# kpreid/all-is-cubes

Hardware: AMD Instinct MI355X
Metric: Mrays/s (higher is better)
Workload: dtype f64

## Files before the change

### all_is_cubes_amd/abi.py

```python
from __future__ import annotations

import ctypes as C
import math
from pathlib import Path
from typing import Optional

import numpy as np

_PKG = Path(__file__).resolve().parent
LIB_PATH = _PKG / "libaic_hip.so"

AIC_OK = 0
ERR_NAMES = {1: "AIC_ERR_INVALID", 2: "AIC_ERR_NO_DEVICE", 3: "AIC_ERR_OOM", 4: "AIC_ERR_DEVICE", 5: "AIC_ERR_UNSUPPORTED"}
LAYER_WORLD, LAYER_UI = 0, 1
MAX_IN_FLIGHT = 32
FLAW_UNSUPPORTED, FLAW_NO_BLOOM = 1, 2
FRAME_COUNTERS, FRAME_AUX, FRAME_PIXEL_CENTERS, FRAME_OUT_LINEAR, FRAME_OUT_COLORBUF, FRAME_NO_FEEDBACK = 1, 2, 4, 8, 16, 32
FRAME_BLOOM = 64
FRAME_OUT_SPLIT = 512
RAYS_NO_SKY, RAYS_DEVICE = 128, 256
MAX_RAYS = 2048 * 65535
PIXELS_DEVICE, PIXELS_IN_PLACE = 1, 2
MAX_PIXELS = 2048 * 65535
REPROJECT_KEEP_SPLATS = 1
# ... 35 lines not shown
        t |= ((int(super_shift) + 1) & 31) << TUNE_SUPER_SHIFT
    if variant is not None:
        t |= (int(variant) & 3) << TUNE_VARIANT_SHIFT
    return t

ABI_SYMBOLS = [
    "aic_abi_version", "aic_create", "aic_destroy", "aic_last_error", "aic_device_name", "aic_upload_space",
    "aic_clear_space", "aic_update_cubes", "aic_update_light_volume", "aic_replace_block", "aic_replace_blocks", "aic_compact", "aic_set_options", "aic_set_depth_transform",
    "aic_render", "aic_render_submit", "aic_render_wait", "aic_render_submit_batch", "aic_render_wait_batch", "aic_trace_patches", "aic_trace_rays", "aic_trace_pixels", "aic_pixel_order", "aic_reproject_split", "aic_reproject_geometry", "aic_pick_pixels", "aic_stale_rects", "aic_pick_stale", "aic_pick_stale_cubes", "aic_probe_stale_cube_rects", "aic_find_block_cubes", "aic_pick_stale_blocks", "aic_present_split", "aic_present_geometry", "aic_present_split_lines", "aic_present_lines_scratch", "aic_cursor_wireframe", "aic_cursor_raycast", "aic_set_text_font", "aic_text_geometry", "aic_text_layout", "aic_present_split_text", "aic_export_split", "aic_export_size", "aic_exposure_init", "aic_exposure_rays", "aic_sample_luminance", "aic_exposure_advance", "aic_partition_rows", "aic_assemble_strips", "aic_assemble_strips_async", "aic_assemble_strips_on", "aic_read_aux", "aic_synchronize", "aic_stream", "aic_wait_event", "aic_stream_wait_frame",
    "aic_probe_raycast", "aic_probe_light_lut", "aic_probe_powf", "aic_probe_expf", "aic_probe_bloom",
    "aic_ortho_image_size", "aic_render_orthographic",
    "aic_evaluate_light", "aic_evaluate_light_submit", "aic_evaluate_light_wait", "aic_evaluate_light_poll", "aic_light_cubes_changed", "aic_light_changed_count", "aic_light_changed_take", "aic_read_light_volume", "aic_read_light_cubes", "aic_light_chart", "aic_probe_derived", "aic_probe_log2f", "aic_probe_cube_grid",
    "aic_create_multi", "aic_destroy_multi", "aic_multi_device_count", "aic_multi_context", "aic_multi_last_error", "aic_multi_upload_space",
    "aic_multi_clear_space", "aic_multi_update_cubes", "aic_multi_update_light_volume", "aic_multi_evaluate_light", "aic_multi_light_cubes_changed", "aic_multi_replace_blocks", "aic_multi_set_options", "aic_multi_set_depth_transform",
    "aic_multi_render", "aic_multi_render_submit", "aic_multi_render_wait",
]


class AicError(RuntimeError):

    def __init__(self, code: int, message: str):
        super().__init__(f"{ERR_NAMES.get(code, code)}: {message}")
        self.code = code


class BlockDesc(C.Structure):
    _fields_ = [("resolution", C.c_int32), ("vlo", C.c_int32 * 3), ("vsize", C.c_int32 * 3), ("vox_off", C.c_uint32),
                ("pal_off", C.c_uint32), ("pal_len", C.c_uint32), ("flags", C.c_uint32), ("reserved", C.c_int32)]


class LightParams(C.Structure):
# ... 362 lines not shown
        lib.aic_last_error.argtypes = [C.c_void_p]
        lib.aic_stream.restype = C.c_void_p
        lib.aic_stream.argtypes = [C.c_void_p]
        lib.aic_partition_rows.restype = C.c_uint32
        lib.aic_partition_rows.argtypes = [C.c_uint32, C.POINTER(Partition)]
        lib.aic_upload_space.argtypes = [C.c_void_p, C.c_int, C.POINTER(SpaceDesc)]
        lib.aic_clear_space.argtypes = [C.c_void_p, C.c_int]
        lib.aic_compact.argtypes = [C.c_void_p, C.c_int]
        lib.aic_update_cubes.argtypes = [C.c_void_p, C.c_int, C.c_uint32, C.c_void_p, C.c_void_p, C.c_void_p]
        lib.aic_update_light_volume.argtypes = [C.c_void_p, C.c_int, C.c_void_p]
        lib.aic_replace_block.argtypes = [C.c_void_p, C.c_int, C.c_uint32, C.POINTER(BlockDesc), C.c_void_p, C.c_void_p]
        lib.aic_replace_blocks.argtypes = [C.c_void_p, C.c_int, C.c_uint32, C.c_void_p, C.c_void_p, C.c_void_p, C.c_void_p]
        lib.aic_set_options.argtypes = [C.c_void_p, C.c_int, C.POINTER(Options)]
        lib.aic_set_depth_transform.argtypes = [C.c_void_p, C.POINTER(C.c_double)]
        lib.aic_render.argtypes = [C.c_void_p, C.POINTER(FrameDesc), C.c_void_p, C.c_int, C.POINTER(FrameInfo)]
        lib.aic_render_submit.argtypes = [C.c_void_p, C.POINTER(FrameDesc), C.c_void_p, C.c_uint32]
        lib.aic_render_wait.argtypes = [C.c_void_p, C.c_uint32, C.POINTER(FrameInfo)]
        lib.aic_render_submit_batch.argtypes = [C.c_void_p, C.c_uint32, C.POINTER(FrameDesc), C.POINTER(C.c_void_p), C.c_uint32]
        lib.aic_render_wait_batch.argtypes = [C.c_void_p, C.c_uint32, C.c_uint32, C.POINTER(FrameInfo)]
        lib.aic_trace_patches.argtypes = [C.c_void_p, C.POINTER(FrameDesc), C.c_uint32, C.c_void_p, C.c_void_p, C.c_void_p, C.POINTER(FrameInfo)]
        lib.aic_trace_rays.argtypes = [C.c_void_p, C.c_int, C.c_uint32, C.c_void_p, C.c_uint32, C.c_float, C.c_void_p, C.c_void_p, C.POINTER(FrameInfo)]
        lib.aic_trace_pixels.argtypes = [C.c_void_p, C.POINTER(FrameDesc), C.c_uint32, C.c_void_p, C.c_uint32, C.c_void_p, C.c_void_p, C.POINTER(FrameInfo)]
        lib.aic_reproject_split.argtypes = [C.c_void_p, C.POINTER(ReprojectDesc), C.c_void_p, C.c_void_p, C.POINTER(ReprojectInfo)]
        lib.aic_pick_pixels.argtypes = [C.c_void_p, C.POINTER(PickDesc), C.c_void_p, C.c_void_p, C.POINTER(PickInfo)]
        lib.aic_pick_stale.argtypes = [C.c_void_p, C.POINTER(StaleDesc), C.c_void_p, C.c_void_p, C.c_void_p, C.POINTER(StaleInfo)]
        lib.aic_light_changed_count.argtypes = [C.c_void_p, C.c_int, C.POINTER(C.c_uint64), C.c_void_p]
        lib.aic_light_changed_take.argtypes = [C.c_void_p, C.c_int, C.c_uint32, C.c_void_p, C.POINTER(C.c_uint32)]
        lib.aic_pick_stale_cubes.argtypes = [C.c_void_p, C.POINTER(StaleCubesDesc), C.c_void_p, C.c_void_p, C.c_void_p, C.POINTER(StaleCubesInfo)]
        lib.aic_probe_stale_cube_rects.argtypes = [C.c_void_p, C.POINTER(StaleCubesDesc), C.c_void_p]
        lib.aic_find_block_cubes.argtypes = [C.c_void_p, C.c_int, C.c_uint32, C.c_void_p, C.c_uint32, C.c_void_p, C.POINTER(BlockCubesInfo)]
# ... 270 lines not shown
        out = np.zeros(rows * frame.width * 3, np.uint32) if split else np.zeros((rows, frame.width, 4), np.float32 if floats else np.uint8)
        info = FrameInfo()
        try:
            self._check(self._lib.aic_render(self._h, C.byref(frame), _ptr(out), 0, C.byref(info)))
        finally:
            frame.flags = keep_flags
        aux = None
        if want_aux:
            aux = np.zeros((rows, frame.width), PIXEL_AUX_DTYPE)
            if aux.size:
                self._check(self._lib.aic_read_aux(self._h, _ptr(aux), aux.size))
        if split:
            return {**split_planes(out, rows, frame.width), "info": info, "aux": aux}
        return {"rgba8": out, "info": info, "aux": aux}

    def render_to_device(self, frame: FrameDesc, device_ptr: int) -> FrameInfo:
        info = FrameInfo()
        self._check(self._lib.aic_render(self._h, C.byref(frame), C.c_void_p(device_ptr), 1, C.byref(info)))
        return info

    def trace_patches(self, frame: FrameDesc, rects, want_aux: bool = False):
        r = np.ascontiguousarray(rects, np.float64).reshape(-1, 4)
        out = np.zeros((len(r), 4), np.float32 if frame.flags & (FRAME_OUT_LINEAR | FRAME_OUT_COLORBUF) else np.uint8)
        aux = np.zeros(len(r), PIXEL_AUX_DTYPE) if want_aux else None
        info = FrameInfo()
        self._check(self._lib.aic_trace_patches(self._h, C.byref(frame), len(r), _ptr(r), _ptr(out), _ptr(aux), C.byref(info)))
        return {"rgba8": out, "aux": aux, "info": info}

    def trace_rays(self, layer: int, rays, include_sky: bool = True, flags: int = 0, exposure: float = 1.0, want_aux: bool = False):
        r = np.ascontiguousarray(rays, np.float64).reshape(-1, 6)
# ... 500 lines not shown
```

### all_is_cubes_amd/csrc/aic_abi.cpp

```cpp

#include <hip/hip_runtime.h>

#include <chrono>
#include <cmath>
#include <condition_variable>
#include <mutex>
#include <thread>
#include <cstdio>
#include <cstdlib>
#include <cstring>
#include <initializer_list>
#include <string>
#include <utility>
#include <vector>

#include "../../include/aic_hip.h"
#include "aic_bloom.h"
#include "aic_ctx.h"
#include "aic_device.h"
#include "aic_encode.h"
#include "aic_launch.h"

using namespace aic;

// ... 303 lines not shown
        aic_ctx::FrameSlot &fs = c->slots[i];
        if (fs.stream) (void)hipStreamSynchronize(fs.stream);
        for (auto &sb : fs.sub) sb.release();
        fs.ray_cold.release(); fs.edges.release();
        if (fs.ev0) (void)hipEventDestroy(fs.ev0);
        if (fs.ev1) (void)hipEventDestroy(fs.ev1);
        if (fs.ev2) (void)hipEventDestroy(fs.ev2);
        fs.tile_static.release(); fs.queue_static.release();
        if (i > 0 && fs.stream) (void)hipStreamDestroy(fs.stream);
    }
    for (auto &l : c->layers) l.release();
    c->lut.release(); c->srgb_thr.release(); c->srgb_buckets.release(); c->out.release(); c->aux.release(); c->staging.release(); c->ortho_views.release(); c->reproject_scratch.release(); c->pick_scratch.release(); c->stale_scratch.release(); c->stale_cubes_scratch.release(); c->stale_blocks_scratch.release(); c->stale_blocks_boxes.release(); c->present_scratch.release(); c->lines_scratch.release();
    c->text_atlas.release(); c->text_codes.release(); c->export_counts.release(); c->exposure_scratch.release(); c->cursor_scratch.release();
    for (hipEvent_t ev : c->stale_blocks_ev)
        if (ev) (void)hipEventDestroy(ev);
    if (c->dump) std::fclose(c->dump);
    if (c->upload_stream) (void)hipStreamDestroy(c->upload_stream);
    if (c->stream) (void)hipStreamDestroy(c->stream);
    delete c;
}

const char *aic_last_error(const aic_ctx *c) { return c ? c->err.c_str() : "no context"; }

int aic_device_name(const aic_ctx *c, char *buf, uint32_t buf_len) {
    if (!c || !buf || !buf_len) return AIC_ERR_INVALID;
    std::snprintf(buf, buf_len, "%s", c->devname);
    return AIC_OK;
}

int aic_upload_space(aic_ctx *c, int layer, const aic_space_desc *s) {
// ... 550 lines not shown
```

### all_is_cubes_amd/csrc/aic_ctx.h

```cpp
#pragma once

#include <hip/hip_runtime.h>

#include <chrono>
#include <condition_variable>
#include <cstdio>
#include <initializer_list>
#include <mutex>
#include <string>
#include <thread>
#include <vector>

#include "../../include/aic_hip.h"
#include "aic_device.h"

namespace aic {

template <typename T>
struct DevBuf {
    T *p = nullptr;
    size_t n = 0;
    size_t cap = 0;
    hipError_t ensure(size_t count, bool keep = false, hipStream_t stream = nullptr) {
        if (count <= cap) { n = count; return hipSuccess; }
        size_t new_cap = count + count / 4 + 16;
        T *np_ = nullptr;
        hipError_t e = hipMalloc((void **)&np_, new_cap * sizeof(T));
        if (e != hipSuccess) return e;
        if (keep && p && cap) {
// ... 155 lines not shown
    } ljob;
    struct Switches {
        int tile = 0, macro = 0;
        bool feedback = true;
        bool wait_whole_stream = false;
        uint32_t tiles_per_wave = 0;
        std::string wave_prof;
        bool lines_clear_keys = false;
    } sw;
    DevBuf<unsigned char> stale_scratch;
    DevBuf<unsigned char> cursor_scratch;
    DevBuf<unsigned char> stale_cubes_scratch;
    DevBuf<unsigned char> stale_blocks_scratch;
    DevBuf<int32_t> stale_blocks_boxes;
    hipEvent_t stale_blocks_ev[2] = {nullptr, nullptr};
};

namespace aic {

extern thread_local std::string *tl_err_sink;
int fail(aic_ctx *c, int code, const char *what, hipError_t e = hipSuccess);
int hip_fail(aic_ctx *c, const char *what, hipError_t e);
inline int reject(aic_ctx *c, const char *who, const char *why) { return fail(c, AIC_ERR_INVALID, (std::string(who) + ": " + why).c_str()); }
#define HIP_TRY(ctx, expr)                                    \
    do {                                                      \
        hipError_t e_ = (expr);                               \
        if (e_ != hipSuccess) return hip_fail(ctx, #expr, e_); \
    } while (0)

inline bool valid_layer(int l) { return l == AIC_LAYER_WORLD || l == AIC_LAYER_UI; }

aic_options default_options();
enum DumpTag : uint32_t { DUMP_UPLOAD = 1, DUMP_CLEAR = 2, DUMP_CUBES = 3, DUMP_LIGHT = 4, DUMP_BLOCK = 5, DUMP_OPTIONS = 6, DUMP_FRAME = 7 };
struct DumpPart { const void *p; size_t n; };
void dump_record(aic_ctx *c, uint32_t tag, uint32_t layer, std::initializer_list<DumpPart> parts);
int take_light_spare(aic_ctx *c, Layer &l, int layer, size_t n, int *index);
int quiesce(aic_ctx *c);
int light_job_finish(aic_ctx *c);
constexpr uint32_t kVisibleBitsWords = 2048;
int light_visible_bits(aic_ctx *c, Layer &l, hipStream_t stream, std::vector<uint32_t> *bits);

}
```

### all_is_cubes_amd/csrc/aic_frame.cpp

```cpp

#include <hip/hip_runtime.h>

#include <algorithm>
#include <chrono>
#include <cmath>
#include <cstdio>
#include <cstring>
#include <utility>
#include <vector>

#include "../../include/aic_hip.h"
#include "aic_bloom.h"
#include "aic_ctx.h"
#include "aic_device.h"
#include "aic_launch.h"

using namespace aic;

namespace {

void fill_dev_layer(const Layer &l, const aic_camera &cam, DevLayer *d) {
    std::memset(d, 0, sizeof(*d));
    d->present = l.present ? 1 : 0;
    d->pool = l.pool.p;
// ... 636 lines not shown
}
int finish_listed(aic_ctx *c, uint32_t n, bool to_host, aic_pixel_aux *aux, aic_frame_info *info) {
    const int rc = wait_frame(c, 0, info, to_host);
    if (rc != AIC_OK) return rc;
    if (aux && to_host) HIP_TRY(c, hipMemcpy(aux, c->aux.p, (size_t)n * sizeof(aic_pixel_aux), hipMemcpyDeviceToHost));
    if (info) info->rows_rendered = n;
    return AIC_OK;
}

int submit_in_world_seat(aic_ctx *c, int layer, const aic_frame_desc *f, uint32_t *target, bool allow_aux, const Traced &what) {
    Traced seated = what;
    seated.world_seat = layer;
    return submit_frame(c, f, target, 0, allow_aux, seated);
}

}

extern "C" {

int aic_render(aic_ctx *c, const aic_frame_desc *f, void *out_rgba8, int out_is_device, aic_frame_info *info) {
    if (!c || !f) return fail(c, AIC_ERR_INVALID, "aic_render: bad argument");
    if (info) std::memset(info, 0, sizeof(*info));
    if (const int rc = begin_on_slot0(c, "aic_render")) return rc;
    uint32_t *target = (uint32_t *)out_rgba8;
    const size_t px_words = (f->flags & (AIC_FRAME_OUT_LINEAR | AIC_FRAME_OUT_COLORBUF)) ? 4 : ((f->flags & AIC_FRAME_OUT_SPLIT) ? 3 : 1);
    if (!out_is_device && out_rgba8) {
        const aic_partition part = normalised_partition(*f);
        const size_t npix = (size_t)f->width * (part.part < part.n_parts ? aic_partition_rows(f->height, &part) : 0);
        hipError_t e;
        if (npix && (e = c->out.ensure(npix * px_words)) != hipSuccess) return hip_fail(c, "alloc output", e);
        target = c->out.p;
    }
    int rc = submit_frame(c, f, target, 0, true);
    if (rc != AIC_OK) return rc;
    if (!out_is_device && c->slots[0].npix)
        HIP_TRY(c, hipMemcpyAsync(out_rgba8, c->out.p, c->slots[0].npix * px_words * 4, hipMemcpyDeviceToHost, c->slots[0].stream));
    return wait_frame(c, 0, info, !out_is_device);
}

int aic_ortho_image_size(const int32_t lo[3], const int32_t size[3], int resolution, uint32_t *width, uint32_t *height) {
    if (!lo || !size || !width || !height || !valid_ortho_resolution(resolution) || size[0] < 0 || size[1] < 0 || size[2] < 0) return AIC_ERR_INVALID;
    DevOrthoView v[5];
    multi_ortho(resolution, lo, size, v, width, height);
// ... 212 lines not shown
```

### all_is_cubes_amd/host/aic_host.cpp

```cpp
#include "aic_host.hpp"

#include <algorithm>
#include <cmath>
#include <cstdio>
#include <cstring>

namespace aic::host {

#define MM(t, r, c) ((t).m[((r)-1) * 4 + ((c)-1)])

Mat4 Mat4::then(const Mat4 &o) const {
    Mat4 out;
    for (int r = 1; r <= 4; r++)
        for (int c = 1; c <= 4; c++)
            MM(out, r, c) = MM(*this, r, 1) * MM(o, 1, c) + MM(*this, r, 2) * MM(o, 2, c) + MM(*this, r, 3) * MM(o, 3, c) +
                            MM(*this, r, 4) * MM(o, 4, c);
    return out;
}

bool Mat4::inverse(Mat4 *out) const {
    const double m11 = MM(*this, 1, 1), m12 = MM(*this, 1, 2), m13 = MM(*this, 1, 3), m14 = MM(*this, 1, 4);
    const double m21 = MM(*this, 2, 1), m22 = MM(*this, 2, 2), m23 = MM(*this, 2, 3), m24 = MM(*this, 2, 4);
    const double m31 = MM(*this, 3, 1), m32 = MM(*this, 3, 2), m33 = MM(*this, 3, 3), m34 = MM(*this, 3, 4);
    const double m41 = MM(*this, 4, 1), m42 = MM(*this, 4, 2), m43 = MM(*this, 4, 3), m44 = MM(*this, 4, 4);
// ... 424 lines not shown
    char buf[256];
    const double per = (width && height) ? (double)cubes_traced / ((double)width * height) : 0.0;
    std::snprintf(buf, sizeof(buf), "Traced %llu cubes, %.1f cubes/pixel in %u\xC3\x97%u image", (unsigned long long)cubes_traced, per, width, height);
    return buf;
}

static_assert(sizeof(PackedLight) == 4, "PackedLight is a 4-byte texel");

HipRtRenderer::HipRtRenderer(std::shared_ptr<StandardCameras> cameras, SizePolicy size_policy, int device_id)
    : cameras_(std::move(cameras)), size_policy_(std::move(size_policy)), world_camera_(GraphicsOptions(), Viewport::with_scale(1.0, 1, 1)),
      ui_camera_(GraphicsOptions(), Viewport::with_scale(1.0, 1, 1)) {
    if (!cameras_) throw std::invalid_argument("cameras must not be null");
    int status = 0;
    ctx_ = aic_create(device_id, &status);
    if (!ctx_) throw RenderError(status, status == AIC_ERR_NO_DEVICE ? "no usable HIP device (MI355X required)" : "aic_create failed");
}
HipRtRenderer::~HipRtRenderer() { aic_destroy(ctx_); }

void HipRtRenderer::check(int rc, const char *what) {
    if (rc != AIC_OK) throw RenderError(rc, std::string(what) + ": " + aic_last_error(ctx_));
}
Viewport HipRtRenderer::modified_viewport() const { return size_policy_ ? size_policy_(cameras_->viewport) : cameras_->viewport; }
std::string HipRtRenderer::device_name() const {
    char buf[256];
    aic_device_name(ctx_, buf, sizeof(buf));
    return buf;
}
void *HipRtRenderer::stream() const { return aic_stream(ctx_); }

void HipRtRenderer::upload_full(int layer, const Space &space) {
    aic_space_desc d;
    std::memset(&d, 0, sizeof(d));
// ... 157 lines not shown
}

static ImageInfo to_info(const aic_frame_info &fi, uint32_t w, uint32_t h) {
    ImageInfo i;
    i.cubes_traced = fi.cubes_traced; i.n_outer = fi.n_outer; i.n_inner = fi.n_inner; i.n_hits = fi.n_hits; i.n_light = fi.n_light;
    i.kernel_ms = fi.kernel_ms; i.total_ms = fi.total_ms; i.width = w; i.height = h; i.rows_rendered = fi.rows_rendered;
    return i;
}

Rendering HipRtRenderer::draw_rgba(const std::string &info_text) {
    aic_frame_desc f = make_frame();
    if (bloom_) f.flags |= AIC_FRAME_BLOOM;
    Rendering r;
    r.width = f.width;
    r.height = f.height;
    r.data.assign((size_t)f.width * f.height * 4, 0);
    aic_frame_info fi;
    check(aic_render(ctx_, &f, r.data.data(), 0, &fi), "aic_render");
    r.info = to_info(fi, f.width, f.height);
    if (fi.flaws & AIC_FLAW_UNSUPPORTED) r.flaws |= Flaws::UNSUPPORTED;
    if (fi.flaws & AIC_FLAW_NO_BLOOM) r.flaws |= Flaws::NO_BLOOM;
    if (had_cursor_) r.flaws |= Flaws::NO_CURSOR;
    if (!info_text.empty() && world_camera_.options().debug_info_text && f.width && f.height) {
        uint8_t black[4], white[4];
        const float k0[3] = {0.f, 0.f, 0.f}, k1[3] = {1.f, 1.f, 1.f};
        const float paint_exposure = cam_override_ ? cam_override_exposure_ : world_camera_.exposure();
        encode_paint(world_camera_, paint_exposure, k0, black);
        encode_paint(world_camera_, paint_exposure, k1, white);
        draw_info_text(r.data.data(), f.width, f.height, black, white, info_text);
    }
    return r;
}

// ... 662 lines not shown
```

### all_is_cubes_amd/host/aic_host.hpp

```cpp
#pragma once

#include <array>
#include <cstdint>
#include <cstring>
#include <functional>
#include <limits>
#include <memory>
#include <optional>
#include <set>
#include <stdexcept>
#include <string>
#include <vector>

#include "../../include/aic_hip.h"

namespace aic::host {

struct Vec3 {
    double x = 0, y = 0, z = 0;
};
struct Quat {
    double i = 0, j = 0, k = 0, r = 1;
};
struct Mat4 {
// ... 210 lines not shown

struct ImageInfo {
    uint64_t cubes_traced = 0;
    uint64_t n_outer = 0, n_inner = 0, n_hits = 0, n_light = 0;
    float kernel_ms = 0, total_ms = 0;
    uint32_t width = 0, height = 0, rows_rendered = 0;
    std::string status_text() const;
};
struct SplitRendering {
    uint32_t width = 0, height = 0;
    std::vector<uint16_t> color;
    std::vector<float> depth;
    uint16_t flaws = 0;
    ImageInfo info;
};
struct Rendering {
    uint32_t width = 0, height = 0;
    std::vector<uint8_t> data;
    uint16_t flaws = 0;
    ImageInfo info;
};

void draw_info_text(uint8_t *rgba, uint32_t width, uint32_t height, const uint8_t outline[4], const uint8_t foreground[4], const std::string &text);
constexpr uint32_t kInfoTextCell[3] = {9, 18, 1};
std::vector<uint8_t> info_text_font_atlas();
void encode_paint(const class Camera &camera, float exposure, const float rgb[3], uint8_t out[4]);

struct UiViewState {
    std::shared_ptr<Space> space;
    ViewTransform view_transform;
    float backdrop[4] = {0, 0, 0, 0};
    GraphicsOptions graphics_options;
};
// ... 166 lines not shown
  private:
    struct LayerState {
        std::shared_ptr<Space> space;
        std::shared_ptr<SpaceRendererTodo> todo;
        GraphicsOptions options;
        bool options_valid = false;
    };
    bool sync_space(int layer, const std::shared_ptr<Space> &space, const GraphicsOptions &options);
    void upload_full(int layer, const Space &space);
    void check(int rc, const char *what);
    aic_present_desc present_desc(uint32_t out_width, uint32_t out_height, uint32_t flags) const;
    aic_frame_desc make_frame() const;
    std::shared_ptr<StandardCameras> cameras_;
    SizePolicy size_policy_;
    aic_ctx *ctx_ = nullptr;
    LayerState layers_[2];
    bool cam_override_ = false;
    double cam_override_inv_[16] = {0};
    float cam_override_exposure_ = 1.0f;
    bool had_cursor_ = false;
    std::vector<aic_line_vertex> cursor_lines_;
    aic_lines_desc lines_desc(const std::vector<aic_line_vertex> *lines) const;
    bool text_font_set_ = false;
    std::vector<uint8_t> text_codes_;
    aic_text_desc text_desc(const std::string &info_text);
    bool bloom_ = false;
    uint64_t pick_cursor_ = 0, pick_skip_unknown_ = 0;
    uint64_t pick_skip_stale_ = 0;
    std::vector<std::array<int32_t, 6>> changed_boxes_;
    std::vector<std::array<int32_t, 6>> changed_cube_boxes_;
// ... 78 lines not shown
```

### all_is_cubes_amd/host/py_module.cpp

```cpp
#include <pybind11/functional.h>
#include <pybind11/numpy.h>
#include <pybind11/pybind11.h>
#include <pybind11/stl.h>

#include <cstring>

#include "aic_host.hpp"

namespace py = pybind11;
using namespace aic::host;

static Vec3 v3(const std::array<double, 3> &a) { return Vec3{a[0], a[1], a[2]}; }
static std::array<double, 3> a3(const Vec3 &v) { return {v.x, v.y, v.z}; }
static py::array_t<double> mat(const Mat4 &m) {
    py::array_t<double> out({4, 4});
    std::memcpy(out.mutable_data(), m.m, sizeof(m.m));
    return out;
}

PYBIND11_MODULE(_host, m) {
    m.doc() = "C++ host mirror of the all-is-cubes raytracer interface above the MI355X C ABI";

    py::register_exception<RenderError>(m, "RenderError");

// ... 192 lines not shown
                      [](UiViewState &u, const std::array<float, 4> &b) { for (int i = 0; i < 4; i++) u.backdrop[i] = b[i]; });
    py::class_<StandardCameras, std::shared_ptr<StandardCameras>>(m, "StandardCameras")
        .def(py::init([]() { return std::make_shared<StandardCameras>(); }))
        .def_readwrite("graphics_options", &StandardCameras::graphics_options).def_readwrite("viewport", &StandardCameras::viewport)
        .def_readwrite("world_space", &StandardCameras::world_space).def_readwrite("world_view_transform", &StandardCameras::world_view_transform)
        .def_readwrite("measured_exposure", &StandardCameras::measured_exposure).def_readwrite("ui", &StandardCameras::ui);

    py::class_<ImageInfo>(m, "ImageInfo")
        .def_readonly("cubes_traced", &ImageInfo::cubes_traced).def_readonly("n_outer", &ImageInfo::n_outer).def_readonly("n_inner", &ImageInfo::n_inner)
        .def_readonly("n_hits", &ImageInfo::n_hits).def_readonly("n_light", &ImageInfo::n_light).def_readonly("kernel_ms", &ImageInfo::kernel_ms)
        .def_readonly("total_ms", &ImageInfo::total_ms).def_readonly("width", &ImageInfo::width).def_readonly("height", &ImageInfo::height)
        .def_readonly("rows_rendered", &ImageInfo::rows_rendered).def("status_text", &ImageInfo::status_text);
    py::class_<Rendering>(m, "Rendering")
        .def_readonly("width", &Rendering::width).def_readonly("height", &Rendering::height).def_readonly("flaws", &Rendering::flaws)
        .def_readonly("info", &Rendering::info)
        .def_property_readonly("data", [](const Rendering &r) {
            py::array_t<uint8_t> a({(py::ssize_t)r.height, (py::ssize_t)r.width, (py::ssize_t)4});
            if (!r.data.empty()) std::memcpy(a.mutable_data(), r.data.data(), r.data.size());
            return a;
        });

    py::class_<SplitRendering>(m, "SplitRendering")
        .def_readonly("width", &SplitRendering::width).def_readonly("height", &SplitRendering::height).def_readonly("flaws", &SplitRendering::flaws)
        .def_readonly("info", &SplitRendering::info)
        .def_property_readonly("color_f16_bits", [](const SplitRendering &r) {
            py::array_t<uint16_t> a({(py::ssize_t)r.height, (py::ssize_t)r.width, (py::ssize_t)4});
            if (!r.color.empty()) std::memcpy(a.mutable_data(), r.color.data(), r.color.size() * 2);
            return a;
        })
        .def_property_readonly("depth", [](const SplitRendering &r) {
            py::array_t<float> a({(py::ssize_t)r.height, (py::ssize_t)r.width});
            if (!r.depth.empty()) std::memcpy(a.mutable_data(), r.depth.data(), r.depth.size() * 4);
            return a;
        });
// ... 391 lines not shown
```

### include/aic_hip.h

```cpp
#ifndef AIC_HIP_H
#define AIC_HIP_H

#include <stdint.h>

#ifdef __cplusplus
extern "C" {
#endif

#define AIC_ABI_VERSION 3

#define AIC_OK 0
#define AIC_ERR_INVALID 1
#define AIC_ERR_NO_DEVICE 2
#define AIC_ERR_OOM 3
#define AIC_ERR_DEVICE 4
#define AIC_ERR_UNSUPPORTED 5

#define AIC_LAYER_WORLD 0
#define AIC_LAYER_UI 1

#define AIC_FLAW_UNSUPPORTED 1u
#define AIC_FLAW_NO_BLOOM 2u

#define AIC_BLOCK_ONE 1u
// ... 118 lines not shown

int aic_upload_space(aic_ctx *ctx, int layer, const aic_space_desc *space);
int aic_clear_space(aic_ctx *ctx, int layer);
int aic_update_cubes(aic_ctx *ctx, int layer, uint32_t n, const int32_t *xyz, const uint16_t *block_index,
                     const uint8_t *light);
int aic_update_light_volume(aic_ctx *ctx, int layer, const uint8_t *light);
int aic_replace_block(aic_ctx *ctx, int layer, uint32_t index, const aic_block_desc *desc, const uint16_t *voxels,
                      const float *palette);
int aic_replace_blocks(aic_ctx *ctx, int layer, uint32_t n, const uint32_t *indices, const aic_block_desc *descs,
                       const uint16_t *const *voxels, const float *const *palettes);
int aic_compact(aic_ctx *ctx, int layer);
int aic_set_options(aic_ctx *ctx, int layer, const aic_options *options);
int aic_set_depth_transform(aic_ctx *ctx, const double zw[4]);

int aic_render(aic_ctx *ctx, const aic_frame_desc *frame, void *out_rgba8, int out_is_device, aic_frame_info *info);
#define AIC_MAX_IN_FLIGHT 32u
int aic_render_submit(aic_ctx *ctx, const aic_frame_desc *frame, void *out_device, uint32_t slot);
int aic_render_wait(aic_ctx *ctx, uint32_t slot, aic_frame_info *info);
int aic_render_submit_batch(aic_ctx *ctx, uint32_t n_frames, const aic_frame_desc *frames, void *const *out_devices, uint32_t slot);
int aic_render_wait_batch(aic_ctx *ctx, uint32_t slot, uint32_t n_frames, aic_frame_info *infos);
int aic_trace_patches(aic_ctx *ctx, const aic_frame_desc *frame, uint32_t n, const double *rects, void *out_rgba8,
                      aic_pixel_aux *aux, aic_frame_info *info);
#define AIC_RAYS_NO_SKY 128u
#define AIC_RAYS_DEVICE 256u
int aic_trace_rays(aic_ctx *ctx, int layer, uint32_t n, const double *rays, uint32_t flags, float exposure, void *out, aic_pixel_aux *aux,
                   aic_frame_info *info);
#define AIC_PIXELS_DEVICE 1u
#define AIC_PIXELS_IN_PLACE 2u
int aic_trace_pixels(aic_ctx *ctx, const aic_frame_desc *frame, uint32_t n, const uint32_t *pixels, uint32_t mode, void *out, aic_pixel_aux *aux,
                     aic_frame_info *info);
// ... 329 lines not shown
```

### rust/all-is-cubes-hip/src/ffi.rs

```rust
#![allow(non_camel_case_types, missing_docs, clippy::missing_safety_doc)]

use core::ffi::{c_char, c_int, c_void};

pub const AIC_ABI_VERSION: c_int = 3;
pub const AIC_OK: c_int = 0;
pub const AIC_ERR_INVALID: c_int = 1;
pub const AIC_ERR_NO_DEVICE: c_int = 2;
pub const AIC_ERR_OOM: c_int = 3;
pub const AIC_ERR_DEVICE: c_int = 4;
pub const AIC_ERR_UNSUPPORTED: c_int = 5;
pub const AIC_LAYER_WORLD: c_int = 0;
pub const AIC_LAYER_UI: c_int = 1;
pub const AIC_BLOCK_ONE: u32 = 1;
pub const AIC_BLOCK_AIR: u32 = 2;
pub const AIC_BLOCK_UNSELECTABLE: u32 = 4;
pub const AIC_BLOCK_VOXEL_SELECTABLE: u32 = 8;
pub const AIC_FLAW_UNSUPPORTED: u32 = 1;
pub const AIC_FLAW_NO_BLOOM: u32 = 2;
pub const AIC_FRAME_COUNTERS: u32 = 1;
pub const AIC_FRAME_AUX: u32 = 2;
pub const AIC_FRAME_PIXEL_CENTERS: u32 = 4;
pub const AIC_FRAME_OUT_LINEAR: u32 = 8;
pub const AIC_FRAME_OUT_COLORBUF: u32 = 16;
pub const AIC_FRAME_NO_FEEDBACK: u32 = 32;
// ... 6 lines not shown
pub const AIC_REPROJECT_KEEP_SPLATS: u32 = 1;
pub const AIC_REPROJECT_MAX_LEVELS: u32 = 12;
pub const AIC_PRESENT_OUT_F16: u32 = 1;
pub const AIC_PRESENT_MAX_PIXELS: u64 = 2147483648;
pub const AIC_LINES_DEVICE: u32 = 1;
pub const AIC_TEXT_DEVICE: u32 = 1;
pub const AIC_LINES_MAX: u32 = 1048576;
pub const AIC_STALE_DEPTH_TEST: u32 = 1;
pub const AIC_STALE_MAX_RECTS: u32 = 4096;
pub const AIC_STALE_DEPTH_BEHIND: u32 = 2;
pub const AIC_CURSOR_MAX_LINES: u32 = 28;
pub const AIC_CURSOR_NO_BLOCK: u32 = 0xFFFF_FFFF;
pub const AIC_EXPOSURE_SAMPLES: u32 = 100;
pub const AIC_EXPOSURE_RAYS: u32 = 10;
pub const AIC_MAX_IN_FLIGHT: u32 = 32;
pub const AIC_MULTI_MAX_IN_FLIGHT: u32 = 8;
pub const AIC_TUNE_QUEUES_SHIFT: u32 = 0;
pub const AIC_TUNE_SUPER_SHIFT: u32 = 4;
pub const AIC_TUNE_VARIANT_SHIFT: u32 = 9;
pub const AIC_VARIANT_AUTO: u32 = 0;
pub const AIC_VARIANT_PLAIN: u32 = 1;
pub const AIC_VARIANT_EXCHANGING: u32 = 2;
pub const AIC_VARIANT_RECORDING: u32 = 3;
pub const AIC_LIGHT_HOOK_SESSION: i32 = 1;
pub const AIC_LIGHT_HOOK_POOL_SHIFT: i32 = 8;

#[repr(C)]
#[derive(Clone, Copy, Debug, Default)]
pub struct aic_block_desc {
    pub resolution: i32,
// ... 425 lines not shown
    pub fn aic_create(device_id: c_int, status: *mut c_int) -> *mut aic_ctx;
    pub fn aic_destroy(ctx: *mut aic_ctx);
    pub fn aic_last_error(ctx: *const aic_ctx) -> *const c_char;
    pub fn aic_abi_version() -> c_int;
    pub fn aic_device_name(ctx: *const aic_ctx, buf: *mut c_char, buf_len: u32) -> c_int;
    pub fn aic_upload_space(ctx: *mut aic_ctx, layer: c_int, space: *const aic_space_desc) -> c_int;
    pub fn aic_clear_space(ctx: *mut aic_ctx, layer: c_int) -> c_int;
    pub fn aic_update_cubes(ctx: *mut aic_ctx, layer: c_int, n: u32, xyz: *const i32, block_index: *const u16, light: *const u8) -> c_int;
    pub fn aic_update_light_volume(ctx: *mut aic_ctx, layer: c_int, light: *const u8) -> c_int;
    pub fn aic_replace_block(ctx: *mut aic_ctx, layer: c_int, index: u32, desc: *const aic_block_desc, voxels: *const u16, palette: *const f32) -> c_int;
    pub fn aic_replace_blocks(ctx: *mut aic_ctx, layer: c_int, n: u32, indices: *const u32, descs: *const aic_block_desc, voxels: *const *const u16, palettes: *const *const f32) -> c_int;
    pub fn aic_compact(ctx: *mut aic_ctx, layer: c_int) -> c_int;
    pub fn aic_set_options(ctx: *mut aic_ctx, layer: c_int, options: *const aic_options) -> c_int;
    pub fn aic_set_depth_transform(ctx: *mut aic_ctx, zw: *const f64) -> c_int;
    pub fn aic_render(ctx: *mut aic_ctx, frame: *const aic_frame_desc, out_rgba8: *mut c_void, out_is_device: c_int, info: *mut aic_frame_info) -> c_int;
    pub fn aic_render_submit(ctx: *mut aic_ctx, frame: *const aic_frame_desc, out_device: *mut c_void, slot: u32) -> c_int;
    pub fn aic_render_wait(ctx: *mut aic_ctx, slot: u32, info: *mut aic_frame_info) -> c_int;
    pub fn aic_render_submit_batch(ctx: *mut aic_ctx, n_frames: u32, frames: *const aic_frame_desc, out_devices: *const *mut c_void, slot: u32) -> c_int;
    pub fn aic_render_wait_batch(ctx: *mut aic_ctx, slot: u32, n_frames: u32, infos: *mut aic_frame_info) -> c_int;
    pub fn aic_trace_patches(ctx: *mut aic_ctx, frame: *const aic_frame_desc, n: u32, rects: *const f64, out_rgba8: *mut c_void, aux: *mut aic_pixel_aux, info: *mut aic_frame_info) -> c_int;
    pub fn aic_partition_rows(height: u32, partition: *const aic_partition) -> u32;
    pub fn aic_assemble_strips(ctx: *mut aic_ctx, gathered_device: *const c_void, out_device: *mut c_void, width: u32, height: u32, strip_rows: u32, n_parts: u32) -> c_int;
    pub fn aic_assemble_strips_async(ctx: *mut aic_ctx, gathered_device: *const c_void, out_device: *mut c_void, width: u32, height: u32, strip_rows: u32, n_parts: u32) -> c_int;
    pub fn aic_assemble_strips_on(ctx: *mut aic_ctx, gathered_device: *const c_void, out_device: *mut c_void, width: u32, height: u32, strip_rows: u32, n_parts: u32, hip_stream: *mut c_void) -> c_int;
    pub fn aic_trace_rays(ctx: *mut aic_ctx, layer: c_int, n: u32, rays: *const f64, flags: u32, exposure: f32, out: *mut c_void, aux: *mut aic_pixel_aux, info: *mut aic_frame_info) -> c_int;
    pub fn aic_trace_pixels(ctx: *mut aic_ctx, frame: *const aic_frame_desc, n: u32, pixels: *const u32, mode: u32, out: *mut c_void, aux: *mut aic_pixel_aux, info: *mut aic_frame_info) -> c_int;
    pub fn aic_reproject_split(ctx: *mut aic_ctx, desc: *const aic_reproject_desc, src_device: *const c_void, dst_device: *mut c_void, info: *mut aic_reproject_info) -> c_int;
    pub fn aic_reproject_geometry(width: u32, height: u32, levels: *mut u32, t0: *mut u32, scratch_bytes: *mut u64) -> c_int;
    pub fn aic_pick_pixels(ctx: *mut aic_ctx, desc: *const aic_pick_desc, order_device: *const u32, pixels_out_device: *mut u32, info: *mut aic_pick_info) -> c_int;
    pub fn aic_stale_rects(view_projection: *const f64, width: u32, height: u32, n_boxes: u32, boxes: *const i32, expand: i32, out: *mut aic_stale_rect) -> c_int;
// ... 95 lines not shown
```

Baseline: 6596.

## Render frames into a pinned host ring and hand them out zero-copy

Adds aic_render_host, which copies the device frame straight into a pool of up to 16 reusable hipHostMalloc'd buffers. The C++ renderer and the Python binding then expose that buffer without copying, with release tied to object lifetime. This removes the pageable staging copy, the per-frame vector allocation and zero-fill, and the extra memcpy into a numpy array. In exchange it adds buffer-lifetime bookkeeping, a hard cap on held frames, and a fallback to pageable memory if pinning fails.

```diff
diff --git a/all_is_cubes_amd/abi.py b/all_is_cubes_amd/abi.py
--- a/all_is_cubes_amd/abi.py
+++ b/all_is_cubes_amd/abi.py
@@ -73,7 +73,9 @@
     "aic_create_multi", "aic_destroy_multi", "aic_multi_device_count", "aic_multi_context", "aic_multi_last_error", "aic_multi_upload_space",
     "aic_multi_clear_space", "aic_multi_update_cubes", "aic_multi_update_light_volume", "aic_multi_evaluate_light", "aic_multi_light_cubes_changed", "aic_multi_replace_blocks", "aic_multi_set_options", "aic_multi_set_depth_transform",
     "aic_multi_render", "aic_multi_render_submit", "aic_multi_render_wait",
+    "aic_render_host", "aic_host_frame_release",
 ]
+HOST_FRAMES_MAX = 16
 
 
 class AicError(RuntimeError):
@@ -466,6 +468,8 @@
         lib.aic_set_options.argtypes = [C.c_void_p, C.c_int, C.POINTER(Options)]
         lib.aic_set_depth_transform.argtypes = [C.c_void_p, C.POINTER(C.c_double)]
         lib.aic_render.argtypes = [C.c_void_p, C.POINTER(FrameDesc), C.c_void_p, C.c_int, C.POINTER(FrameInfo)]
+        lib.aic_render_host.argtypes = [C.c_void_p, C.POINTER(FrameDesc), C.POINTER(C.c_void_p), C.POINTER(C.c_uint64), C.POINTER(FrameInfo)]
+        lib.aic_host_frame_release.argtypes = [C.c_void_p, C.c_void_p]
         lib.aic_render_submit.argtypes = [C.c_void_p, C.POINTER(FrameDesc), C.c_void_p, C.c_uint32]
         lib.aic_render_wait.argtypes = [C.c_void_p, C.c_uint32, C.POINTER(FrameInfo)]
         lib.aic_render_submit_batch.argtypes = [C.c_void_p, C.c_uint32, C.POINTER(FrameDesc), C.POINTER(C.c_void_p), C.c_uint32]
@@ -766,6 +770,19 @@
             return {**split_planes(out, rows, frame.width), "info": info, "aux": aux}
         return {"rgba8": out, "info": info, "aux": aux}
 
+    def render_host(self, frame: FrameDesc):
+        ptr, nbytes, info = C.c_void_p(), C.c_uint64(), FrameInfo()
+        self._check(self._lib.aic_render_host(self._h, C.byref(frame), C.byref(ptr), C.byref(nbytes), C.byref(info)))
+        if not ptr.value:
+            return {"ptr": None, "bytes": np.zeros(0, np.uint8), "info": info}
+        view = np.ctypeslib.as_array(C.cast(ptr, C.POINTER(C.c_uint8)), shape=(nbytes.value,))
+        return {"ptr": ptr.value, "bytes": view, "info": info}
+
+    def host_frame_release(self, ptr) -> None:
+        rc = self._lib.aic_host_frame_release(self._h, C.c_void_p(ptr))
+        if rc != 0:
+            raise AicError(rc, "aic_host_frame_release: not a host frame this context handed out and still holds")
+
     def render_to_device(self, frame: FrameDesc, device_ptr: int) -> FrameInfo:
         info = FrameInfo()
         self._check(self._lib.aic_render(self._h, C.byref(frame), C.c_void_p(device_ptr), 1, C.byref(info)))
diff --git a/all_is_cubes_amd/csrc/aic_abi.cpp b/all_is_cubes_amd/csrc/aic_abi.cpp
--- a/all_is_cubes_amd/csrc/aic_abi.cpp
+++ b/all_is_cubes_amd/csrc/aic_abi.cpp
@@ -341,6 +341,7 @@
     c->text_atlas.release(); c->text_codes.release(); c->export_counts.release(); c->exposure_scratch.release(); c->cursor_scratch.release();
     for (hipEvent_t ev : c->stale_blocks_ev)
         if (ev) (void)hipEventDestroy(ev);
+    c->host_ring.free_all(host_ring_alloc());
     if (c->dump) std::fclose(c->dump);
     if (c->upload_stream) (void)hipStreamDestroy(c->upload_stream);
     if (c->stream) (void)hipStreamDestroy(c->stream);
diff --git a/all_is_cubes_amd/csrc/aic_ctx.h b/all_is_cubes_amd/csrc/aic_ctx.h
--- a/all_is_cubes_amd/csrc/aic_ctx.h
+++ b/all_is_cubes_amd/csrc/aic_ctx.h
@@ -5,6 +5,7 @@
 #include <chrono>
 #include <condition_variable>
 #include <cstdio>
+#include <cstdlib>
 #include <initializer_list>
 #include <mutex>
 #include <string>
@@ -13,6 +14,7 @@
 
 #include "../../include/aic_hip.h"
 #include "aic_device.h"
+#include "aic_host_ring.h"
 
 namespace aic {
 
@@ -198,6 +200,8 @@
     DevBuf<unsigned char> stale_blocks_scratch;
     DevBuf<int32_t> stale_blocks_boxes;
     hipEvent_t stale_blocks_ev[2] = {nullptr, nullptr};
+    HostFrameRing host_ring;
+    std::mutex host_ring_mu;
 };
 
 namespace aic {
@@ -212,6 +216,15 @@
         if (e_ != hipSuccess) return hip_fail(ctx, #expr, e_); \
     } while (0)
 
+inline const HostRingAlloc &host_ring_alloc() {
+    static const HostRingAlloc a = {
+        [](size_t n) -> void * { void *p = nullptr; return hipHostMalloc(&p, n, hipHostMallocDefault) == hipSuccess ? p : nullptr; },
+        [](void *p) { (void)hipHostFree(p); },
+        [](size_t n) -> void * { return std::malloc(n); },
+        [](void *p) { std::free(p); }};
+    return a;
+}
+
 inline bool valid_layer(int l) { return l == AIC_LAYER_WORLD || l == AIC_LAYER_UI; }
 
 aic_options default_options();
diff --git a/all_is_cubes_amd/csrc/aic_frame.cpp b/all_is_cubes_amd/csrc/aic_frame.cpp
--- a/all_is_cubes_amd/csrc/aic_frame.cpp
+++ b/all_is_cubes_amd/csrc/aic_frame.cpp
@@ -674,19 +674,82 @@
     return submit_frame(c, f, target, 0, allow_aux, seated);
 }
 
+size_t frame_px_words(const aic_frame_desc &f) { return (f.flags & (AIC_FRAME_OUT_LINEAR | AIC_FRAME_OUT_COLORBUF)) ? 4 : ((f.flags & AIC_FRAME_OUT_SPLIT) ? 3 : 1); }
+size_t frame_part_pixels(const aic_frame_desc &f) {
+    const aic_partition part = normalised_partition(f);
+    return (size_t)f.width * (part.part < part.n_parts ? aic_partition_rows(f.height, &part) : 0);
+}
+
+int host_frame_acquire(aic_ctx *c, size_t bytes, void **p, bool *pinned) {
+    std::lock_guard<std::mutex> lk(c->host_ring_mu);
+    HostFrameRing::Status st;
+    const int slot = c->host_ring.acquire(host_ring_alloc(), bytes, &st);
+    if (slot < 0) {
+        if (st == HostFrameRing::kAllHeld)
+            return reject(c, "aic_render_host", "AIC_HOST_FRAMES_MAX (16) host frames are held: release one with aic_host_frame_release first");
+        return fail(c, AIC_ERR_OOM, "aic_render_host: no host memory for the frame, pinned or pageable");
+    }
+    *p = c->host_ring.slot((uint32_t)slot).p;
+    *pinned = c->host_ring.slot((uint32_t)slot).pinned;
+    return AIC_OK;
+}
+bool host_frame_release(aic_ctx *c, const void *p) {
+    std::lock_guard<std::mutex> lk(c->host_ring_mu);
+    return c->host_ring.release(p);
+}
+
 }
 
 extern "C" {
+
+int aic_render_host(aic_ctx *c, const aic_frame_desc *f, void **out_host, uint64_t *out_bytes, aic_frame_info *info) {
+    if (!c || !f || !out_host || !out_bytes) return fail(c, AIC_ERR_INVALID, "aic_render_host: bad argument");
+    *out_host = nullptr;
+    *out_bytes = 0;
+    if (info) std::memset(info, 0, sizeof(*info));
+    if (const int rc = begin_on_slot0(c, "aic_render_host")) return rc;
+    const size_t px_words = frame_px_words(*f), npix = frame_part_pixels(*f);
+    void *host = nullptr;
+    bool pinned = true;
+    if (npix) {
+        const hipError_t e = c->out.ensure(npix * px_words);
+        if (e != hipSuccess) return hip_fail(c, "alloc output", e);
+        if (const int rc = host_frame_acquire(c, npix * px_words * 4, &host, &pinned)) return rc;
+    }
+    int rc = submit_frame(c, f, c->out.p, 0, true);
+    const size_t bytes = rc == AIC_OK ? c->slots[0].npix * px_words * 4 : 0;
+    if (rc == AIC_OK && bytes) {
+        const hipError_t e = bytes <= npix * px_words * 4 ? hipMemcpyAsync(host, c->out.p, bytes, hipMemcpyDeviceToHost, c->slots[0].stream) : hipErrorInvalidValue;
+        if (e != hipSuccess) {
+            (void)wait_frame(c, 0, nullptr, true);
+            rc = hip_fail(c, "copy the frame to its host slot", e);
+        }
+    }
+    if (rc == AIC_OK) rc = wait_frame(c, 0, info, true);
+    if (rc != AIC_OK || !bytes) {
+        if (host) (void)host_frame_release(c, host);
+        return rc;
+    }
+    if (!pinned) c->err = "aic_render_host: hipHostMalloc failed for the frame's slot; delivered through pageable memory (a staged copy)";
+    *out_host = host;
+    *out_bytes = bytes;
+    return AIC_OK;
+}
+
+int aic_host_frame_release(aic_ctx *c, void *host_frame) {
+    if (!c) return AIC_ERR_INVALID;
+    if (!host_frame) return AIC_OK;
+    return host_frame_release(c, host_frame) ? AIC_OK : AIC_ERR_INVALID;
+}
 
 int aic_render(aic_ctx *c, const aic_frame_desc *f, void *out_rgba8, int out_is_device, aic_frame_info *info) {
     if (!c || !f) return fail(c, AIC_ERR_INVALID, "aic_render: bad argument");
     if (info) std::memset(info, 0, sizeof(*info));
     if (const int rc = begin_on_slot0(c, "aic_render")) return rc;
     uint32_t *target = (uint32_t *)out_rgba8;
-    const size_t px_words = (f->flags & (AIC_FRAME_OUT_LINEAR | AIC_FRAME_OUT_COLORBUF)) ? 4 : ((f->flags & AIC_FRAME_OUT_SPLIT) ? 3 : 1);
+    const size_t px_words = frame_px_words(*f);
     if (!out_is_device && out_rgba8) {
-        const aic_partition part = normalised_partition(*f);
-        const size_t npix = (size_t)f->width * (part.part < part.n_parts ? aic_partition_rows(f->height, &part) : 0);
+        const size_t npix = frame_part_pixels(*f);
         hipError_t e;
         if (npix && (e = c->out.ensure(npix * px_words)) != hipSuccess) return hip_fail(c, "alloc output", e);
         target = c->out.p;
diff --git a/all_is_cubes_amd/csrc/aic_host_ring.h b/all_is_cubes_amd/csrc/aic_host_ring.h
--- /dev/null
+++ b/all_is_cubes_amd/csrc/aic_host_ring.h
@@ -0,0 +1,76 @@
+#pragma once
+
+#include <cstddef>
+#include <cstdint>
+
+namespace aic {
+
+constexpr uint32_t kHostRingMax = 16;
+
+struct HostRingAlloc {
+    void *(*alloc_pinned)(size_t bytes);
+    void (*free_pinned)(void *p);
+    void *(*alloc_pageable)(size_t bytes);
+    void (*free_pageable)(void *p);
+};
+
+class HostFrameRing {
+  public:
+    struct Slot {
+        void *p = nullptr;
+        size_t cap = 0;
+        bool held = false, pinned = false;
+    };
+    enum Status { kOk = 0, kAllHeld = 1, kNoMemory = 2 };
+
+    int acquire(const HostRingAlloc &a, size_t bytes, Status *status) {
+        *status = kOk;
+        int pick = -1;
+        for (uint32_t i = 0; i < n_ && pick < 0; i++)
+            if (!slots_[i].held && slots_[i].cap >= bytes) pick = (int)i;
+        if (pick < 0) {
+            for (uint32_t i = 0; i < n_ && pick < 0; i++)
+                if (!slots_[i].held) pick = (int)i;
+            if (pick < 0) {
+                if (n_ == kHostRingMax) { *status = kAllHeld; return -1; }
+                pick = (int)n_;
+            }
+            bool pinned = true;
+            void *p = a.alloc_pinned(bytes);
+            if (!p) { pinned = false; p = a.alloc_pageable(bytes); }
+            if (!p) { *status = kNoMemory; return -1; }
+            Slot &s = slots_[pick];
+            drop(a, s);
+            s.p = p; s.cap = bytes; s.pinned = pinned;
+            if ((uint32_t)pick == n_) n_++;
+        }
+        slots_[pick].held = true;
+        return pick;
+    }
+    bool release(const void *p) {
+        for (uint32_t i = 0; i < n_; i++)
+            if (slots_[i].held && slots_[i].p == p) { slots_[i].held = false; return true; }
+        return false;
+    }
+    void free_all(const HostRingAlloc &a) {
+        for (uint32_t i = 0; i < n_; i++) drop(a, slots_[i]);
+        n_ = 0;
+    }
+    uint32_t size() const { return n_; }
+    const Slot &slot(uint32_t i) const { return slots_[i]; }
+    uint32_t held() const {
+        uint32_t k = 0;
+        for (uint32_t i = 0; i < n_; i++) k += slots_[i].held ? 1u : 0u;
+        return k;
+    }
+
+  private:
+    static void drop(const HostRingAlloc &a, Slot &s) {
+        if (s.p) (s.pinned ? a.free_pinned : a.free_pageable)(s.p);
+        s = Slot();
+    }
+    Slot slots_[kHostRingMax];
+    uint32_t n_ = 0;
+};
+
+}
diff --git a/all_is_cubes_amd/host/aic_host.cpp b/all_is_cubes_amd/host/aic_host.cpp
--- a/all_is_cubes_amd/host/aic_host.cpp
+++ b/all_is_cubes_amd/host/aic_host.cpp
@@ -462,8 +462,9 @@
     int status = 0;
     ctx_ = aic_create(device_id, &status);
     if (!ctx_) throw RenderError(status, status == AIC_ERR_NO_DEVICE ? "no usable HIP device (MI355X required)" : "aic_create failed");
-}
-HipRtRenderer::~HipRtRenderer() { aic_destroy(ctx_); }
+    ctx_owner_ = std::shared_ptr<aic_ctx>(ctx_, [](aic_ctx *c) { aic_destroy(c); });
+}
+HipRtRenderer::~HipRtRenderer() = default;
 
 void HipRtRenderer::check(int rc, const char *what) {
     if (rc != AIC_OK) throw RenderError(rc, std::string(what) + ": " + aic_last_error(ctx_));
@@ -651,9 +652,11 @@
     Rendering r;
     r.width = f.width;
     r.height = f.height;
-    r.data.assign((size_t)f.width * f.height * 4, 0);
     aic_frame_info fi;
-    check(aic_render(ctx_, &f, r.data.data(), 0, &fi), "aic_render");
+    void *slot = nullptr;
+    uint64_t bytes = 0;
+    check(aic_render_host(ctx_, &f, &slot, &bytes, &fi), "aic_render_host");
+    if (slot) r.data = FrameBytes(ctx_owner_, slot, (size_t)bytes);
     r.info = to_info(fi, f.width, f.height);
     if (fi.flaws & AIC_FLAW_UNSUPPORTED) r.flaws |= Flaws::UNSUPPORTED;
     if (fi.flaws & AIC_FLAW_NO_BLOOM) r.flaws |= Flaws::NO_BLOOM;
diff --git a/all_is_cubes_amd/host/aic_host.hpp b/all_is_cubes_amd/host/aic_host.hpp
--- a/all_is_cubes_amd/host/aic_host.hpp
+++ b/all_is_cubes_amd/host/aic_host.hpp
@@ -248,9 +248,58 @@
     uint16_t flaws = 0;
     ImageInfo info;
 };
+class FrameBytes {
+  public:
+    FrameBytes() = default;
+    FrameBytes(std::shared_ptr<aic_ctx> ctx, void *slot, size_t bytes) : ctx_(std::move(ctx)), p_(static_cast<uint8_t *>(slot)), n_(bytes) {}
+    FrameBytes(const FrameBytes &o) : own_(o.begin(), o.end()) { adopt_own(); }
+    FrameBytes(FrameBytes &&o) noexcept { take(std::move(o)); }
+    FrameBytes &operator=(const FrameBytes &o) {
+        if (this != &o) { std::vector<uint8_t> copy(o.begin(), o.end()); reset(); own_ = std::move(copy); adopt_own(); }
+        return *this;
+    }
+    FrameBytes &operator=(FrameBytes &&o) noexcept {
+        if (this != &o) { reset(); take(std::move(o)); }
+        return *this;
+    }
+    ~FrameBytes() { reset(); }
+    void assign(size_t n, uint8_t value) { reset(); own_.assign(n, value); adopt_own(); }
+    uint8_t *data() { return p_; }
+    const uint8_t *data() const { return p_; }
+    size_t size() const { return n_; }
+    bool empty() const { return n_ == 0; }
+    uint8_t &operator[](size_t i) { return p_[i]; }
+    const uint8_t &operator[](size_t i) const { return p_[i]; }
+    uint8_t *begin() { return p_; }
+    uint8_t *end() { return p_ + n_; }
+    const uint8_t *begin() const { return p_; }
+    const uint8_t *end() const { return p_ + n_; }
+
+  private:
+    void adopt_own() { p_ = own_.empty() ? nullptr : own_.data(); n_ = own_.size(); }
+    void take(FrameBytes &&o) {
+        ctx_ = std::move(o.ctx_);
+        own_ = std::move(o.own_);
+        p_ = ctx_ ? o.p_ : nullptr;
+        n_ = ctx_ ? o.n_ : 0;
+        if (!ctx_) adopt_own();
+        o.ctx_.reset(); o.own_.clear(); o.p_ = nullptr; o.n_ = 0;
+    }
+    void reset() {
+        if (ctx_ && p_) (void)aic_host_frame_release(ctx_.get(), p_);
+        ctx_.reset();
+        own_.clear();
+        p_ = nullptr;
+        n_ = 0;
+    }
+    std::shared_ptr<aic_ctx> ctx_;
+    uint8_t *p_ = nullptr;
+    size_t n_ = 0;
+    std::vector<uint8_t> own_;
+};
 struct Rendering {
     uint32_t width = 0, height = 0;
-    std::vector<uint8_t> data;
+    FrameBytes data;
     uint16_t flaws = 0;
     ImageInfo info;
 };
@@ -447,6 +496,7 @@
     std::shared_ptr<StandardCameras> cameras_;
     SizePolicy size_policy_;
     aic_ctx *ctx_ = nullptr;
+    std::shared_ptr<aic_ctx> ctx_owner_;
     LayerState layers_[2];
     bool cam_override_ = false;
     double cam_override_inv_[16] = {0};
diff --git a/all_is_cubes_amd/host/py_module.cpp b/all_is_cubes_amd/host/py_module.cpp
--- a/all_is_cubes_amd/host/py_module.cpp
+++ b/all_is_cubes_amd/host/py_module.cpp
@@ -230,10 +230,11 @@
     py::class_<Rendering>(m, "Rendering")
         .def_readonly("width", &Rendering::width).def_readonly("height", &Rendering::height).def_readonly("flaws", &Rendering::flaws)
         .def_readonly("info", &Rendering::info)
-        .def_property_readonly("data", [](const Rendering &r) {
-            py::array_t<uint8_t> a({(py::ssize_t)r.height, (py::ssize_t)r.width, (py::ssize_t)4});
-            if (!r.data.empty()) std::memcpy(a.mutable_data(), r.data.data(), r.data.size());
-            return a;
+        .def_property_readonly("data", [](py::object self) {
+            Rendering &r = self.cast<Rendering &>();
+            const std::vector<py::ssize_t> shape = {(py::ssize_t)r.height, (py::ssize_t)r.width, (py::ssize_t)4};
+            if (r.data.empty() || r.data.size() != (size_t)r.height * r.width * 4) return py::array_t<uint8_t>(shape);
+            return py::array_t<uint8_t>(shape, r.data.data(), self);
         });
 
     py::class_<SplitRendering>(m, "SplitRendering")
diff --git a/include/aic_hip.h b/include/aic_hip.h
--- a/include/aic_hip.h
+++ b/include/aic_hip.h
@@ -156,6 +156,9 @@
 int aic_set_depth_transform(aic_ctx *ctx, const double zw[4]);
 
 int aic_render(aic_ctx *ctx, const aic_frame_desc *frame, void *out_rgba8, int out_is_device, aic_frame_info *info);
+#define AIC_HOST_FRAMES_MAX 16u
+int aic_render_host(aic_ctx *ctx, const aic_frame_desc *frame, void **out_host, uint64_t *out_bytes, aic_frame_info *info);
+int aic_host_frame_release(aic_ctx *ctx, void *host_frame);
 #define AIC_MAX_IN_FLIGHT 32u
 int aic_render_submit(aic_ctx *ctx, const aic_frame_desc *frame, void *out_device, uint32_t slot);
 int aic_render_wait(aic_ctx *ctx, uint32_t slot, aic_frame_info *info);
diff --git a/profiles/scripts_r08/ab_figures.py b/profiles/scripts_r08/ab_figures.py
--- /dev/null
+++ b/profiles/scripts_r08/ab_figures.py
@@ -0,0 +1,34 @@
+import glob
+import json
+import os
+import statistics
+import sys
+
+
+def figures(d):
+    s = d.get("single_frame") or {}
+    sec = ((d.get("secondary") or {}).get("s256") or {})
+    crit = d.get("criterion_equivalent") or {}
+    out = {"fps_with_readback": d.get("fps_with_readback"), "value": d.get("value"), "ms_per_step": d.get("ms_per_step"),
+           "single_frame_warm_ms": s.get("single_frame_warm_ms"), "single_frame_cold_ms": s.get("single_frame_cold_ms"),
+           "streamed_batched.ms_per_step": (d.get("streamed_batched") or {}).get("ms_per_step"), "secondary.s256.ms_per_step": sec.get("ms_per_step")}
+    for k, v in crit.items():
+        if isinstance(v, dict):
+            out[f"criterion.{k}.median_us"] = v.get("median_us")
+            out[f"criterion.{k}.min_us"] = v.get("min_us")
+    return {k: v for k, v in out.items() if v is not None}
+
+
+if sys.argv[1] == "--summary":
+    rows = {}
+    for f in sorted(glob.glob(os.path.join(sys.argv[2], "*.json"))):
+        name, tree, r = os.path.basename(f)[:-5].rsplit("_", 2)
+        for k, v in figures(json.loads(open(f).read())).items():
+            rows.setdefault((name, k), {}).setdefault(tree, []).append((int(r), v))
+    for (name, k), trees in sorted(rows.items()):
+        for tree, vals in sorted(trees.items()):
+            v = [x for _, x in sorted(vals)]
+            print(f"{name:10s} {k:34s} {tree:7s} median {statistics.median(v):.4f} spread {max(v) - min(v):.4f}  rounds {' '.join(f'{x:.4f}' for x in v)}")
+else:
+    f, name, tree, r = sys.argv[1:5]
+    print(f"{name:10s} {tree:7s} r{r} " + " ".join(f"{k} {v}" for k, v in figures(json.loads(open(f).read())).items()), flush=True)
diff --git a/rust/all-is-cubes-hip/src/ffi.rs b/rust/all-is-cubes-hip/src/ffi.rs
--- a/rust/all-is-cubes-hip/src/ffi.rs
+++ b/rust/all-is-cubes-hip/src/ffi.rs
@@ -44,6 +44,7 @@
 pub const AIC_EXPOSURE_SAMPLES: u32 = 100;
 pub const AIC_EXPOSURE_RAYS: u32 = 10;
 pub const AIC_MAX_IN_FLIGHT: u32 = 32;
+pub const AIC_HOST_FRAMES_MAX: u32 = 16;
 pub const AIC_MULTI_MAX_IN_FLIGHT: u32 = 8;
 pub const AIC_TUNE_QUEUES_SHIFT: u32 = 0;
 pub const AIC_TUNE_SUPER_SHIFT: u32 = 4;
@@ -499,6 +500,8 @@
     pub fn aic_set_options(ctx: *mut aic_ctx, layer: c_int, options: *const aic_options) -> c_int;
     pub fn aic_set_depth_transform(ctx: *mut aic_ctx, zw: *const f64) -> c_int;
     pub fn aic_render(ctx: *mut aic_ctx, frame: *const aic_frame_desc, out_rgba8: *mut c_void, out_is_device: c_int, info: *mut aic_frame_info) -> c_int;
+    pub fn aic_render_host(ctx: *mut aic_ctx, frame: *const aic_frame_desc, out_host: *mut *mut c_void, out_bytes: *mut u64, info: *mut aic_frame_info) -> c_int;
+    pub fn aic_host_frame_release(ctx: *mut aic_ctx, host_frame: *mut c_void) -> c_int;
     pub fn aic_render_submit(ctx: *mut aic_ctx, frame: *const aic_frame_desc, out_device: *mut c_void, slot: u32) -> c_int;
     pub fn aic_render_wait(ctx: *mut aic_ctx, slot: u32, info: *mut aic_frame_info) -> c_int;
     pub fn aic_render_submit_batch(ctx: *mut aic_ctx, n_frames: u32, frames: *const aic_frame_desc, out_devices: *const *mut c_void, slot: u32) -> c_int;
```

After: 6581. Within noise of the previous version (-0.2%).
